# numtel/ntru-circom

Hardware: AMD Instinct MI355X
Metric: NTRU encrypt+decrypt round trips per second at N=821, q=4096 (higher is better)
Workload: dtype i8

## Files before the change

ntru-circom_amd/csrc/matrix_common.h:

```cpp
#ifndef NTRU_MATRIX_COMMON_H
#define NTRU_MATRIX_COMMON_H

#include "kernels_common.h"

typedef int v4i __attribute__((ext_vector_type(4)));
typedef int v16i __attribute__((ext_vector_type(16)));
typedef unsigned int v2u __attribute__((__vector_size__(2 * sizeof(unsigned int))));
constexpr int ST_AUX = 0;

struct MGeom {
  int N;
  int NT;
  int pitchA;
  int tpitch;
  int ld;
};

enum { M_ENC = 0, M_DEC1 = 1, M_DEC2 = 2, M_DEC1T = 3, M_DEC2P = 4 };

#ifdef NTRU_STAMPS
#define STAMP_SLOTS 24
#define STAMP_BLOCKS 6
static __device__ unsigned long long g_stamps[1024][8][STAMP_BLOCKS][STAMP_SLOTS];
#define STAMP(slot)                                                                                          \
// ... 3 lines not shown
  } while (0)
#define NTRU_STAMPS_READER(name) extern "C" int name(void *dst) { return (int)hipMemcpyFromSymbol(dst, HIP_SYMBOL(g_stamps), sizeof(g_stamps)); }
#else
#define STAMP(slot) do { } while (0)
#define NTRU_STAMPS_READER(name)
#endif


template <class D>
static __device__ __forceinline__ void build_toeplitz_array(u32 *T, const MGeom &g, D digit, int tid, int nthr) {
  const int Y0 = 32 * g.NT - 1;
  for (int x = tid; x < 4 * g.tpitch; x += nthr) {
    const int c = x / g.tpitch, w = x - c * g.tpitch;
    u32 v = 0;
#pragma unroll
    for (int j = 0; j < 4; j++) {
      int idx = (Y0 - (4 * w + c + j)) % g.N;
      idx += idx < 0 ? g.N : 0;
      v |= ((u32)digit(idx) & 0xFFu) << (8 * j);
    }
    T[x] = v;
  }
}

static __device__ __forceinline__ const u32 *frag_lane_base(const u32 *T, const MGeom &g, int lane) {
  const int y0 = 32 * g.NT - 1 - (lane & 31) + 16 * (lane >> 5);
  return T + (y0 & 3) * g.tpitch + (y0 >> 2);
}

static __device__ __forceinline__ v4i and4(v4i a, const u32 (&m)[4]) {
  return (v4i){(int)((u32)a[0] & m[0]), (int)((u32)a[1] & m[1]), (int)((u32)a[2] & m[2]), (int)((u32)a[3] & m[3])};
}

struct NoPause { __device__ __forceinline__ void operator()() const {} };
struct NoDiag { __device__ __forceinline__ void operator()(int) const {} };
template <int MODE, int NT_S, class Epi, class Pause = NoPause, class Diag = NoDiag>
static __device__ __forceinline__ void toeplitz_strip(const unsigned char *__restrict__ st0,
                                                      const unsigned char *__restrict__ st1,
                                                      const u32 *__restrict__ tb0, const u32 *__restrict__ tb1,
                                                      const MGeom &g, int kb0, const u32 (&mlow)[4], Epi epi,
                                                      int stamp_iter = 0, int stamp_base = 0, int pause_ib = 0x7fffffff,
                                                      Pause pause = Pause(), Diag diag = Diag(), int ash = 0) {
  constexpr bool TWO = MODE != M_DEC2 && MODE != M_DEC2P;
  v16i accL[NT_S], accH[NT_S];
  v4i W0[NT_S], W1[NT_S];
  auto load_w = [&](int d, v4i &w0, v4i &w1) {
    const u32 *p = tb0 - 8 * d;
    w0 = (v4i){(int)p[0], (int)p[1], (int)p[2], (int)p[3]};
    if (MODE == M_ENC || MODE == M_DEC1T) {
      const u32 *p1 = tb1 - 8 * d;
      w1 = (v4i){(int)p1[0], (int)p1[1], (int)p1[2], (int)p1[3]};
    } else if (MODE == M_DEC1) {
#pragma unroll
      for (int c = 0; c < 4; c++) w1[c] = (int)(((u32)w0[c] << 6) & 0xC0C0C0C0u);
    } else {
      w1 = w0;
    }
  };
  auto load_a = [&](int ib, v4i &a0, v4i &a1) {
    a0 = *(const v4i *)(st0 + 32 * ib);
    if (MODE == M_ENC) {
#pragma unroll
      for (int c = 0; c < 4; c++) a1[c] = (int)((u32)a0[c] << 5);
    } else if (MODE == M_DEC1 || MODE == M_DEC1T) {
      a1 = *(const v4i *)(st1 + 32 * ib);
    } else {
      a1 = a0;
    }
  };
  auto unpack_a = [&](v4i &a0, v4i &a1) {
    if (MODE == M_DEC2P) {
#pragma unroll
      for (int c = 0; c < 4; c++) a0[c] = (int)(((u32)a0[c] >> ash) & 0x03030303u);
      a1 = a0;
    }
  };
  auto mm = [&](v16i &acc, v4i a0, v4i a1, v4i w0, v4i w1) {
    acc = __builtin_amdgcn_mfma_i32_32x32x32_i8(a0, w0, acc, 0, 0, 0);
    if (TWO) acc = __builtin_amdgcn_mfma_i32_32x32x32_i8(a1, w1, acc, 0, 0, 0);
  };
  auto mm_first = [&](v16i &acc, v4i a0, v4i a1, v4i w0, v4i w1) {
    const v16i zero = {0, 0, 0, 0, 0, 0, 0, 0, 0, 0, 0, 0, 0, 0, 0, 0};
    acc = __builtin_amdgcn_mfma_i32_32x32x32_i8(a0, w0, zero, 0, 0, 0);
    if (TWO) acc = __builtin_amdgcn_mfma_i32_32x32x32_i8(a1, w1, acc, 0, 0, 0);
  };
#pragma unroll
  for (int t = 0; t < NT_S; t++) load_w(kb0 + t, W0[t], W1[t]);
  u32 mhigh[4];
#pragma unroll
  for (int c = 0; c < 4; c++) mhigh[c] = ~mlow[c];
  v4i a0, a1;
  load_a(0, a0, a1);
  unpack_a(a0, a1);
  auto block = [&](int ib, auto kind) {
#pragma unroll
    for (int u = 0; u < NT_S; u++) {
      v4i n0, n1;
      load_a(ib + u + 1, n0, n1);
#pragma unroll
      for (int tt = 1; tt <= NT_S; tt++) {
        const int t = tt % NT_S;
        constexpr int K = decltype(kind)::value;
        const int sl = (t - u + NT_S) % NT_S;
        if (K == 0 || (K == 2 && t > u)) mm(accL[t], a0, a1, W0[sl], W1[sl]);
        else if (K == 1 || (K == 2 && t < u)) mm(accH[t], a0, a1, W0[sl], W1[sl]);
        else {
          mm(accL[t], a0, a1, and4(W0[sl], mlow), and4(W1[sl], mlow));
          mm_first(accH[t], a0, a1, and4(W0[sl], mhigh), and4(W1[sl], mhigh));
        }
      }
      load_w(kb0 - (ib + u + 1), W0[(NT_S - 1 - u) % NT_S], W1[(NT_S - 1 - u) % NT_S]);
      if (decltype(kind)::value == 2) diag(u);
      a0 = n0; a1 = n1;
      unpack_a(a0, a1);
    }
  };
  auto single = [&](int ib, v16i (&acc)[NT_S]) {
    v4i n0, n1;
    load_a(ib + 1, n0, n1);
#pragma unroll
    for (int t = 0; t < NT_S; t++) mm(acc[t], a0, a1, W0[t], W1[t]);
#pragma unroll
    for (int t = NT_S - 1; t > 0; t--) { W0[t] = W0[t - 1]; W1[t] = W1[t - 1]; }
    load_w(kb0 - (ib + 1), W0[0], W1[0]);
    a0 = n0; a1 = n1;
    unpack_a(a0, a1);
  };
  int ib = 0;
  bool paused = false;
  if (kb0 > 0 && g.NT > 0) {
    if (!std::is_same<Pause, NoPause>::value && pause_ib <= 0) { pause(); paused = true; load_a(0, a0, a1); unpack_a(a0, a1); }
    v4i n0, n1;
    load_a(1, n0, n1);
#pragma unroll
    for (int t = 0; t < NT_S; t++) mm_first(accL[t], a0, a1, W0[t], W1[t]);
#pragma unroll
    for (int t = NT_S - 1; t > 0; t--) { W0[t] = W0[t - 1]; W1[t] = W1[t - 1]; }
    load_w(kb0 - 1, W0[0], W1[0]);
    a0 = n0; a1 = n1;
    unpack_a(a0, a1);
    ib = 1;
  } else {
#pragma unroll
    for (int t = 0; t < NT_S; t++)
#pragma unroll
      for (int i = 0; i < 16; i++) accL[t][i] = 0;
  }
  auto maybe_pause = [&](int first, int last) {
    if (!std::is_same<Pause, NoPause>::value && !paused && last >= pause_ib) {
      __builtin_amdgcn_s_setprio(0);
      pause();
      __builtin_amdgcn_s_setprio(3);
      paused = true;
      load_a(first, a0, a1);
      unpack_a(a0, a1);
    }
  };
  __builtin_amdgcn_s_setprio(3);
  for (; ib + NT_S <= kb0; ib += NT_S) { maybe_pause(ib, ib + NT_S - 1); block(ib, std::integral_constant<int, 0>{}); }
  for (; ib < kb0; ib++) { maybe_pause(ib, ib); single(ib, accL); }
  maybe_pause(kb0, kb0 + NT_S - 1);
  block(kb0, std::integral_constant<int, 2>{});
  for (ib = kb0 + NT_S; ib + NT_S <= g.NT; ib += NT_S) { maybe_pause(ib, ib + NT_S - 1); block(ib, std::integral_constant<int, 1>{}); }
  for (; ib < g.NT; ib++) { maybe_pause(ib, ib); single(ib, accH); }
  __builtin_amdgcn_s_setprio(0);
  if (!std::is_same<Pause, NoPause>::value && !paused) pause();
  STAMP(stamp_base);
  epi(accL, accH);
  STAMP(stamp_base + 1);
}

template <int MAXT = 4, class Body>
static __device__ __forceinline__ void for_each_strip(int NT, int wave, Body body, bool all = false) {
  const int rounds = (((NT + MAXT - 1) / MAXT) + WAVES_PER_BLOCK - 1) / WAVES_PER_BLOCK;
  const int n_str = rounds * WAVES_PER_BLOCK, base = NT / n_str, rem = NT % n_str;
  if (!all && 2 * blockIdx.x >= gridDim.x) wave ^= 2;
  for (int rho = 0; rho < rounds; rho++) {
    const int j = rho * WAVES_PER_BLOCK + wave;
    const int nt = base + (j < rem ? 1 : 0);
    if (nt > 0 || all) body(j * base + (j < rem ? j : rem), nt);
  }
}

static __device__ __forceinline__ void diag_low_mask(int lane, u32 (&mlow)[4]) {
  const int r = lane & 31, hh = lane >> 5;
#pragma unroll
  for (int c = 0; c < 4; c++) {
    u32 mk = 0;
#pragma unroll
    for (int jj = 0; jj < 4; jj++) mk |= (r >= 16 * hh + 4 * c + jj) ? (0xFFu << (8 * jj)) : 0u;
    mlow[c] = mk;
  }
}

static __device__ __forceinline__ __amdgpu_buffer_rsrc_t rows_rsrc(const void *p, long bytes) {
  const unsigned long long a = (unsigned long long)p;
  const u32 lo = __builtin_amdgcn_readfirstlane((u32)a), hi = __builtin_amdgcn_readfirstlane((u32)(a >> 32));
  const int n = __builtin_amdgcn_readfirstlane((int)(bytes < 0x7FFFF000L ? bytes : 0x7FFFF000L));
  return __builtin_amdgcn_make_buffer_rsrc((void *)(((unsigned long long)hi << 32) | lo), 0, n, 0x00020000);
}
// ... 58 lines not shown
```

ntru-circom_amd/csrc/matrix_decrypt.hip:

```cpp
#include "matrix_common.h"

template <int GROUPS, bool PACK = false>
static __device__ __forceinline__ void decrypt_m_body(MGeom g, u32 q, u32 p, const int8_t *__restrict__ f,
                                                      const uint8_t *__restrict__ fp,
                                                      const u16 *__restrict__ e, long B,
                                                      uint8_t *__restrict__ value, u16 *__restrict__ quot1,
                                                      u16 *__restrict__ rem1, uint8_t *__restrict__ quot2,
                                                      unsigned long long *__restrict__ packed = nullptr, int pack_os = 0) {
  extern __shared__ __attribute__((aligned(16))) unsigned char lds[];
  const int group = GROUPS == 2 ? __builtin_amdgcn_readfirstlane((int)(threadIdx.x >> 8)) : 0;
  static_assert(!PACK || GROUPS == 1, "fused packOutput is built on the plain four-wave kernel");
  const int M3V = __builtin_amdgcn_readfirstlane(((int)((p - 1) * (p - 1)) * g.N + 4) & ~3);
  const int m3_bytes = GROUPS == 2 ? (M3V + (int)((p - 1) * (p - 1)) * g.N + 1 + 15) & ~15 : 0;
  const int gbytes = 64 * g.pitchA + 256 * g.NT;
  unsigned char *stHi = lds + (GROUPS == 2 ? __builtin_amdgcn_readfirstlane(m3_bytes + group * gbytes) : 0);
  unsigned char *stLo = stHi + 32 * g.pitchA;
  unsigned char *blp = stLo + 32 * g.pitchA;
  u32 *TF = (u32 *)(lds + m3_bytes + GROUPS * gbytes), *TP = TF + 4 * g.tpitch, *TF64 = TP + 4 * g.tpitch;
  unsigned char *lift_lut = (unsigned char *)(TP + 4 * g.tpitch * GROUPS);
  const int pcols = 126 * pack_os + 16, pimg_bytes = (8 * pcols + 15) & ~15;
  unsigned char *pimg = stHi + ((((int)((p - 1) * (p - 1)) * g.N + 4) & ~3) + (int)((p - 1) * (p - 1)) * g.N + 1 + 15 & ~15);
  auto pack_flush = [&](long rbx) {
    const long b0x = rbx << 5;
    const int rows_left = (int)(B - b0x < 32 ? B - b0x : 32);
// ... 82 lines not shown
      u32 cmask[8];
#pragma unroll
      for (int c = 0; c < 8; c++) {
        const int left2 = N - (16 * c16 + 2 * c);
        cmask[c] = qm2 & (left2 >= 2 ? 0xFFFFFFFFu : (left2 == 1 ? 0x0000FFFFu : 0u));
      }
#pragma unroll
      for (int j = 0; j < RPW; j++) {
        const int row = wave + WAVES_PER_BLOCK * j;
        v4i v[2];
        shift_raw<2>(raw[j], sh[j], v);
        u32 x[8];
#pragma unroll
        for (int c = 0; c < 4; c++) { x[c] = (u32)v[0][c]; x[4 + c] = (u32)v[1][c]; }
        u32 lo[4], hi[4];
#pragma unroll
        for (int c = 0; c < 4; c++) {
          const u32 xa = x[2 * c] & cmask[2 * c], xb = x[2 * c + 1] & cmask[2 * c + 1];
          lo[c] = __builtin_amdgcn_perm(xb & 0x007F007Fu, xa & 0x007F007Fu, 0x06040200u);
          hi[c] = __builtin_amdgcn_perm((xb >> 6) & 0x00FE00FEu, (xa >> 6) & 0x00FE00FEu, 0x06040200u);
        }
        if (c16 < nch) {
          *(uint4 *)(stLo + row * g.pitchA + 16 * c16) = make_uint4(lo[0], lo[1], lo[2], lo[3]);
          *(uint4 *)(stHi + row * g.pitchA + 16 * c16) = make_uint4(hi[0], hi[1], hi[2], hi[3]);
        }
      }
    }
    STAMP(2);
    __syncthreads();
    STAMP(3);
    const int lane_off = (lane >> 5) * 4 * LD + (lane & 31);
    sidx = 0;
    constexpr int P1 = GROUPS == 2 ? M_DEC1T : M_DEC1;
    for_each_strip<4>(g.NT, GROUPS == 2 ? wave ^ (2 * group) ^ (2 * blockIdx.x >= gridDim.x ? 2 : 0) : wave, [&](int kb0, int nt) {
      auto epi = [&](auto &lo, auto &hi) {
        constexpr int NTS = sizeof(lo) / sizeof(lo[0]);
        phase();
        long bb = b0;
        asm volatile("" : "+s"(bb));
        const long lf = (B - bb) * LD;
        const __amdgpu_buffer_rsrc_t rs_r1 = rows_rsrc(want_r1 ? rem1 + bb * LD : nullptr, want_r1 ? 2 * lf : 0);
        const __amdgpu_buffer_rsrc_t rs_q1 = rows_rsrc(want_q1 ? quot1 + bb * LD : nullptr, want_q1 ? 2 * lf : 0);
        int voff[NTS];
#pragma unroll
        for (int t = 0; t < NTS; t++) voff[t] = 32 * (kb0 + t) + (lane & 31) < N ? 2 * lane_off : (int)0x80000000;
        auto out = [&](auto wr, auto wq) {
#pragma unroll
          for (int j = 0; j < 4; j++) {
            u32 xs[NTS][4], lv[NTS][4];
#pragma unroll
            for (int ii = 0; ii < 4; ii++) {
              const int i = 4 * j + ii, ro = ii + 8 * j;
#pragma unroll
              for (int t = 0; t < NTS; t++) {
                const u32 x = (u32)(lo[t][i] + hi[t][i]) & (q - 1);
                xs[t][ii] = x;
                const int so = 2 * (ro * LD + 32 * (kb0 + t));
                {
                  if (decltype(wr)::value) __builtin_amdgcn_raw_buffer_store_b16((u16)x, rs_r1, voff[t], so, ST_AUX);
                  if (decltype(wq)::value) __builtin_amdgcn_raw_buffer_store_b16((u16)((u32)(0 - hi[t][i]) & (q - 1)), rs_q1, voff[t], so, ST_AUX);
                }
              }
            }
#pragma unroll
            for (int t = 0; t < NTS; t++)
#pragma unroll
              for (int ii = 0; ii < 4; ii++) lv[t][ii] = lift_lut[xs[t][ii]];
#pragma unroll
            for (int t = 0; t < NTS; t++) {
              const int col = 32 * (kb0 + t) + (lane & 31);
              const u32 pk = lv[t][0] | (lv[t][1] << 2) | (lv[t][2] << 4) | (lv[t][3] << 6);
              blp[((lane >> 5) + 2 * j) * 32 * g.NT + col] = (unsigned char)(col < N ? pk : 0u);
            }
          }
        };
        if (want_r1 && want_q1) out(std::true_type{}, std::true_type{});
        else if (want_r1) out(std::true_type{}, std::false_type{});
        else if (want_q1) out(std::false_type{}, std::true_type{});
        else out(std::false_type{}, std::false_type{});
      };
      switch (nt) {
        case 0: phase(); break;
        case 1: toeplitz_strip<P1, 1>(st0, st1, tbf, tbf64, g, kb0, mlow, epi, stamp_iter, 4 + 2 * sidx); break;
        case 2: toeplitz_strip<P1, 2>(st0, st1, tbf, tbf64, g, kb0, mlow, epi, stamp_iter, 4 + 2 * sidx); break;
        case 3: toeplitz_strip<P1, 3>(st0, st1, tbf, tbf64, g, kb0, mlow, epi, stamp_iter, 4 + 2 * sidx); break;
        default: toeplitz_strip<P1, 4>(st0, st1, tbf, tbf64, g, kb0, mlow, epi, stamp_iter, 4 + 2 * sidx); break;
      }
      sidx++;
      if (sidx < rounds) phase();
    }, GROUPS == 2);
    __syncthreads();
    STAMP(8);
    if (PACK) pack_wipe();
    if (GROUPS == 1) build_m3(tid0, BLOCK_THREADS, N);
    if (GROUPS == 1) {
      constexpr int RPW = 32 / WAVES_PER_BLOCK;
      u32 pv[RPW][4];
#pragma unroll
      for (int j = 0; j < RPW; j++) {
        const int row = wave + WAVES_PER_BLOCK * j, rgb = 2 * (row >> 3) + ((row >> 2) & 1);
        const u32 *src = (const u32 *)(blp + rgb * 32 * g.NT);
#pragma unroll
        for (int it = 0; it < 4; it++) pv[j][it] = src[(lane + 64 * it) < 8 * g.NT ? lane + 64 * it : 0];
      }
#pragma unroll
      for (int j = 0; j < RPW; j++) {
        const int row = wave + WAVES_PER_BLOCK * j, sh = 2 * (row & 3);
#pragma unroll
        for (int it = 0; it < 4; it++)
          if (lane + 64 * it < 8 * g.NT) *(u32 *)(stLo + row * g.pitchA + 4 * (lane + 64 * it)) = (pv[j][it] >> sh) & 0x03030303u;
      }
    }
    STAMP(9);
    if (GROUPS == 1) __syncthreads();
    STAMP(10);
    constexpr int P2 = GROUPS == 2 ? M_DEC2P : M_DEC2;
    const unsigned char *a2 = GROUPS == 2 ? blp + ((lane & 31) >> 2) * 32 * g.NT + 16 * (lane >> 5) : st0;
    const int ash = 2 * (lane & 3);
    sidx = 0;
// ... 124 lines not shown
```

ntru-circom_amd/csrc/matrix_encrypt.hip:

```cpp
#include "matrix_common.h"

template <int MAXT, bool DMA>
static __device__ __forceinline__ void encrypt_m_body(MGeom g, u32 q, const u16 *__restrict__ h,
                                                      const uint8_t *__restrict__ r,
                                                      const uint8_t *__restrict__ m, long B,
                                                      u16 *__restrict__ e, u16 *__restrict__ quotE) {
  extern __shared__ __attribute__((aligned(16))) unsigned char lds[];
  auto wg_barrier = [&]() {
    if (DMA) asm volatile("s_waitcnt lgkmcnt(0)\n\ts_barrier" ::: "memory");
    else __syncthreads();
  };
  u32 *T0 = (u32 *)lds, *T1 = T0 + 4 * g.tpitch;
  unsigned char *stA = (unsigned char *)(T1 + 4 * g.tpitch);
  unsigned char *mimg = stA + 32 * g.pitchA;
  const int tid0 = threadIdx.x & (BLOCK_THREADS - 1), lane0 = tid0 & 63, wave = __builtin_amdgcn_readfirstlane(tid0 >> 6);
  const int hthr = (int)(q >> 1) - 65;
  auto hs_of = [&](int i) { int hv = (int)(h[i] & (q - 1)); return hv > hthr ? hv - (int)q : hv; };
  if (q <= 4096) {
    build_toeplitz_array(T0, g, [&](int i) { return (int)(h[i] & (q - 1)) & 127; }, (int)threadIdx.x, BLOCK_THREADS);
    build_toeplitz_array(T1, g, [&](int i) { return ((int)(h[i] & (q - 1)) >> 7) * 4; }, (int)threadIdx.x, BLOCK_THREADS);
  } else {
    build_toeplitz_array(T0, g, [&](int i) { const int hs = hs_of(i); return ((hs + 64) & 127) - 64; }, (int)threadIdx.x, BLOCK_THREADS);
    build_toeplitz_array(T1, g, [&](int i) { const int hs = hs_of(i); const int d0 = ((hs + 64) & 127) - 64; return ((hs - d0) >> 7) * 4; }, (int)threadIdx.x, BLOCK_THREADS);
  }
  const bool want_q = quotE != nullptr;
  const long nrb = (B + 31) >> 5;
  int sidx = 0, stamp_iter = -1;
  const long stride = (long)gridDim.x, iters = (nrb + stride - 1) / stride;
  const int rounds = (((g.NT + MAXT - 1) / MAXT) + WAVES_PER_BLOCK - 1) / WAVES_PER_BLOCK;
  auto dma_r = [&](long rbx, int lane) {
    const long b0x = rbx << 5 < B ? rbx << 5 : B;
    const unsigned long long a = (unsigned long long)(r + b0x * g.ld);
    const int a0 = (int)(a & 3);
    const __amdgpu_buffer_rsrc_t rs = rows_rsrc((const void *)(a & ~3ULL), ((B - b0x) * g.ld + a0 + 3) & ~3L);
#pragma unroll
    for (int j = 0; j < 32 / WAVES_PER_BLOCK; j++) {
      const int row = wave + WAVES_PER_BLOCK * j, ro = a0 + row * g.ld;
      if (lane < (((ro & 3) + g.N + 15) >> 4))
        __builtin_amdgcn_raw_ptr_buffer_load_lds(rs, (__attribute__((address_space(3))) void *)(stA + row * g.pitchA), 16,
                                                 (ro & ~3) + 16 * lane, 0, 0, 0);
    }
  };
  auto dma_m = [&](long rbx, int tid) {
    const long b0x = rbx << 5 < B ? rbx << 5 : B;
    const unsigned long long a = (unsigned long long)(m + b0x * g.ld);
    const int a0 = (int)(a & 3);
    const __amdgpu_buffer_rsrc_t rs = rows_rsrc((const void *)(a & ~3ULL), ((B - b0x) * g.ld + a0 + 3) & ~3L);
    const int npc = (a0 + 32 * g.ld + 15) >> 4;
#pragma unroll
    for (int j = 0; j < 8; j++)
      if (tid + j * BLOCK_THREADS < npc)
        __builtin_amdgcn_raw_ptr_buffer_load_lds(rs, (__attribute__((address_space(3))) void *)(mimg + 16 * (wave * 64 + j * BLOCK_THREADS)), 16,
                                                 16 * (tid + j * BLOCK_THREADS), 0, 0, 0);
  };
  if (DMA) {
    dma_r((long)blockIdx.x < nrb ? (long)blockIdx.x : nrb, lane0);
    __builtin_amdgcn_s_waitcnt(0);
  }
  for (long it = 0; it < iters; it++) {
    long rb = (long)blockIdx.x + it * stride;
    rb = rb < nrb ? rb : nrb;
    long rb_next = (long)blockIdx.x + (it + 1) * stride;
    rb_next = rb_next < nrb ? rb_next : nrb;
    stamp_iter++;
    STAMP(0);
    int lane = lane0, N = g.N, LD = g.ld, tid = tid0;
    asm volatile("" : "+v"(lane), "+s"(N), "+s"(LD), "+v"(tid));
    const u32 *tb0 = frag_lane_base(T0, g, lane), *tb1 = frag_lane_base(T1, g, lane);
    const unsigned char *st0 = stA + (lane & 31) * g.pitchA + 16 * (lane >> 5);
    u32 mlow[4];
    diag_low_mask(lane, mlow);
    const long b0 = rb << 5 < B ? rb << 5 : B, left = (B - b0) * LD;
    const AlignedSrc src_r = aligned_src(r + b0 * LD, left), src_m = aligned_src(m + b0 * LD, left);
    constexpr int RPW = 32 / WAVES_PER_BLOCK;
    const int shm = __builtin_amdgcn_readfirstlane(src_m.a0);
    RawChunks<1> in_r[RPW], in_m[8];
    if (!DMA) {
#pragma unroll
      for (int j = 0; j < RPW; j++) {
        const int pos0 = src_r.a0 + (wave + WAVES_PER_BLOCK * j) * LD;
        in_r[j] = load_raw<1>(src_r, pos0 + 16 * lane, 0);
      }
#pragma unroll
      for (int j = 0; j < 8; j++) {
        const int i = tid * 16 + j * BLOCK_THREADS * 16;
        in_m[j] = load_raw<1>(src_m, src_m.a0 + i, 0);
      }
    }
    wg_barrier();
    STAMP(1);
    const int a0m = DMA ? __builtin_amdgcn_readfirstlane((int)((unsigned long long)(m + b0 * LD) & 3)) : 0;
    if (DMA) {
      dma_m(rb, tid);
      const int a0r = (int)((unsigned long long)(r + b0 * LD) & 3);
      const v4i mk = col_mask16(16 * lane, N);
      int s4[RPW];
#pragma unroll
      for (int j = 0; j < RPW; j++) {
        const int row = wave + WAVES_PER_BLOCK * j;
        const unsigned char *slot = stA + row * g.pitchA + 16 * (lane < 2 * g.NT ? lane : 0);
        in_r[j].c[0] = *(const v4i *)slot;
        in_r[j].tail = *(const u32 *)(slot + 16);
        s4[j] = __builtin_amdgcn_readfirstlane((a0r + row * LD) & 3);
      }
// ... 4 lines not shown
        shift_raw<1>(in_r[j], s4[j], v);
        if (lane < 2 * g.NT) *(v4i *)(stA + row * g.pitchA + 16 * lane) = v[0] & mk;
      }
    } else {
      const v4i mk = col_mask16(16 * lane, N);
#pragma unroll
      for (int j = 0; j < RPW; j++) {
        const int row = wave + WAVES_PER_BLOCK * j;
        v4i v[1];
        shift_raw<1>(in_r[j], src_r.a0 + row * LD, v);
        if (lane < 2 * g.NT) *(v4i *)(stA + row * g.pitchA + 16 * lane) = v[0] & mk;
      }
      STAMP(16);
#pragma unroll
      for (int j = 0; j < 8; j++) {
        const int i = tid * 16 + j * BLOCK_THREADS * 16;
        v4i v[1];
        shift_raw<1>(in_m[j], shm, v);
        if (i < 32 * LD) *(v4i *)(mimg + i) = v[0];
      }
    }
    STAMP(2);
    wg_barrier();
    STAMP(3);
    sidx = 0;
    auto epi_sync = [&]() {
      if (!DMA) return;
      if (sidx == 0) __builtin_amdgcn_s_waitcnt((7 << 4) | (15 << 8));
      if (sidx == 0 || sidx == rounds - 1) wg_barrier();
      if (sidx == rounds - 1 && it + 1 < iters) dma_r(rb_next, lane);
    };
    const bool dma_now = DMA && it + 1 < iters;
    for_each_strip<MAXT>(g.NT, DMA ? wave ^ (2 * (int)blockIdx.x >= (int)gridDim.x ? 2 : 0) : wave, [&](int kb0, int nt) {
      const int lane_off = (lane >> 5) * 4 * LD + (lane & 31);
      auto epi = [&](auto &lo, auto &hi) {
        constexpr int NTS = sizeof(lo) / sizeof(lo[0]);
        epi_sync();
        long bb = b0;
        asm volatile("" : "+s"(bb));
        const long lf = (B - bb) * LD;
        const __amdgpu_buffer_rsrc_t rs_e = rows_rsrc(e + bb * LD, 2 * lf);
        const __amdgpu_buffer_rsrc_t rs_q = rows_rsrc(want_q ? quotE + bb * LD : e + bb * LD, 2 * lf);
        const unsigned char *m_l = mimg + a0m + 32 * kb0 + lane_off;
        int voff[NTS];
#pragma unroll
        for (int t = 0; t < NTS; t++) voff[t] = 32 * (kb0 + t) + (lane & 31) < N ? 2 * lane_off : (int)0x80000000;
        const int pv0 = 32 * kb0 + lane;
        auto out = [&](auto wq) {
#pragma unroll
          for (int j = 0; j < 4; j++) {
            u32 mv[NTS][4];
#pragma unroll
            for (int t = 0; t < NTS; t++)
#pragma unroll
              for (int ii = 0; ii < 4; ii++) mv[t][ii] = m_l[(8 * j + ii) * LD + 32 * t];
            u32 ev[NTS][4], qv[NTS][4];
#pragma unroll
            for (int t = 0; t < NTS; t++)
#pragma unroll
              for (int ii = 0; ii < 4; ii++) {
                ev[t][ii] = (u32)(lo[t][4 * j + ii] + hi[t][4 * j + ii] + (int)mv[t][ii]) & (q - 1);
                qv[t][ii] = (u32)(0 - hi[t][4 * j + ii]) & (q - 1);
              }
#pragma unroll
            for (int t = 0; t + 1 < NTS; t += 2) {
              const int pvoff = pv0 + 32 * t < N ? 2 * lane : (int)0x80000000;
#pragma unroll
              for (int ii = 0; ii < 4; ii++) {
                const auto se = __builtin_amdgcn_permlane32_swap(ev[t][ii], ev[t + 1][ii], false, false);
                const int so = 2 * ((8 * j + ii) * LD + 32 * (kb0 + t));
                {
                  __builtin_amdgcn_raw_buffer_store_b16((u16)se[0], rs_e, pvoff, so, ST_AUX);
                  __builtin_amdgcn_raw_buffer_store_b16((u16)se[1], rs_e, pvoff, so + 8 * LD, ST_AUX);
                  if (decltype(wq)::value) {
                    const auto sq = __builtin_amdgcn_permlane32_swap(qv[t][ii], qv[t + 1][ii], false, false);
                    __builtin_amdgcn_raw_buffer_store_b16((u16)sq[0], rs_q, pvoff, so, ST_AUX);
                    __builtin_amdgcn_raw_buffer_store_b16((u16)sq[1], rs_q, pvoff, so + 8 * LD, ST_AUX);
                  }
                }
              }
            }
            if (NTS & 1) {
              constexpr int t = NTS - 1;
              const int so = 2 * (8 * j * LD + 32 * (kb0 + t));
              {
#pragma unroll
                for (int ii = 0; ii < 4; ii++) {
                  __builtin_amdgcn_raw_buffer_store_b16((u16)ev[t][ii], rs_e, voff[t], so + 2 * ii * LD, ST_AUX);
                  if (decltype(wq)::value) __builtin_amdgcn_raw_buffer_store_b16((u16)qv[t][ii], rs_q, voff[t], so + 2 * ii * LD, ST_AUX);
                }
              }
            }
          }
          constexpr int S = 16 * NTS * (decltype(wq)::value ? 2 : 1), K = S < 63 ? S : 63;
          if (DMA && dma_now && sidx == rounds - 1) __builtin_amdgcn_s_waitcnt((K & 15) | (7 << 4) | (15 << 8) | ((K >> 4) << 14));
        };
        if (want_q) out(std::true_type{}); else out(std::false_type{});
      };
      switch (nt) {
        case 0:
          epi_sync();
          if (DMA && sidx == rounds - 1) __builtin_amdgcn_s_waitcnt((7 << 4) | (15 << 8));
          break;
        case 1: toeplitz_strip<M_ENC, 1>(st0, st0, tb0, tb1, g, kb0, mlow, epi, stamp_iter, 4 + 2 * sidx); break;
        case 2: toeplitz_strip<M_ENC, 2>(st0, st0, tb0, tb1, g, kb0, mlow, epi, stamp_iter, 4 + 2 * sidx); break;
        case 3: toeplitz_strip<M_ENC, 3>(st0, st0, tb0, tb1, g, kb0, mlow, epi, stamp_iter, 4 + 2 * sidx); break;
        case 4: toeplitz_strip<M_ENC, 4>(st0, st0, tb0, tb1, g, kb0, mlow, epi, stamp_iter, 4 + 2 * sidx); break;
        default: break;
      }
      sidx++;
    }, DMA);
  }
}

__global__ __launch_bounds__(BLOCK_THREADS, 2) void k_encrypt_m(MGeom g, u32 q, const u16 *__restrict__ h,
                                                             const uint8_t *__restrict__ r,
                                                             const uint8_t *__restrict__ m, long B,
                                                             u16 *__restrict__ e, u16 *__restrict__ quotE) {
  encrypt_m_body<4, false>(g, q, h, r, m, B, e, quotE);
}

__global__ __launch_bounds__(BLOCK_THREADS, 2) void k_encrypt_md(MGeom g, u32 q, const u16 *__restrict__ h,
                                                              const uint8_t *__restrict__ r,
                                                              const uint8_t *__restrict__ m, long B,
                                                              u16 *__restrict__ e, u16 *__restrict__ quotE) {
  encrypt_m_body<4, true>(g, q, h, r, m, B, e, quotE);
}

NTRU_STAMPS_READER(ntru_debug_read_stamps_enc)

int ntru_launch_encrypt_matrix(ntru_engine *eng, int N, int q, int ld, const uint16_t *d_h, const uint8_t *d_r, const uint8_t *d_m,
                               int64_t B, uint16_t *d_e, uint16_t *d_quotE) {
  MGeom mg;
  if (!make_mgeom(eng, N, q, ld, &mg)) return NTRU_NOT_TAKEN;
  const size_t lds = (size_t)32 * mg.tpitch + (size_t)32 * mg.pitchA + (((size_t)32 * ld + 15) & ~(size_t)15) + 16;
  const long nrb = (long)((B + 31) / 32);
  if (lds > 160 * 1024) return NTRU_NOT_TAKEN;
  const bool rows_dword_aligned = (ld & 3) == 0 && ((uintptr_t)d_r & 3) == 0, img_dword_aligned = (ld & 3) == 0 && ((uintptr_t)d_m & 3) == 0;
  const bool dma_fits = (N + 3 <= 1024 || (rows_dword_aligned && N <= 1024)) && (32 * ld + 3 <= 32768 || (img_dword_aligned && 32 * ld <= 32768));
  const bool md = eng->path != 4 && dma_fits;
  snprintf(eng->last_kernel, sizeof eng->last_kernel, md ? "k_encrypt_md" : "k_encrypt_m");
  return launch_resident(eng, md ? k_encrypt_md : k_encrypt_m, nrb, BLOCK_THREADS, lds, mg, (u32)q, d_h, d_r, d_m, (long)B, d_e, d_quotE);
}
```

Before: 275.8 million.

## Add 16x16x64 MFMA tile form to Toeplitz strip and use it in grouped decrypt

Adds a T16 variant of the Toeplitz strip that issues four 16x16x64 int8 MFMAs per step instead of two 32x32x32 ones. It uses lane-dependent stage and key-fragment bases, a per-lane triangular diagonal mask and a permlane16 swap before the epilogue to restore the row layout. The epilogues are generalized for the new row mapping. The two-group decrypt path now uses this form, while the encrypt kernels keep the 32x32 form. A standalone microbenchmark compares the two MFMA shapes for throughput and power.

```diff
diff --git a/bench_micro/mfma_shape_energy.hip b/bench_micro/mfma_shape_energy.hip
--- /dev/null
+++ b/bench_micro/mfma_shape_energy.hip
@@ -0,0 +1,124 @@
+#include <hip/hip_runtime.h>
+#include <cstdio>
+#include <cstdlib>
+#include <cstring>
+#include <vector>
+#define CK(x) do { hipError_t e_ = (x); if (e_ != hipSuccess) { printf("HIP error %s at %d\n", hipGetErrorString(e_), __LINE__); exit(1);} } while (0)
+typedef int v4i __attribute__((ext_vector_type(4)));
+typedef int v16i __attribute__((ext_vector_type(16)));
+constexpr int PITCH = 32 * 26 + 16, NSTEP = 24;
+constexpr int A_BYTES = 64 * PITCH, T_DW = 1024, LDS_BYTES = A_BYTES + 2 * 4 * T_DW;
+
+template <int SHAPE>
+__global__ __launch_bounds__(512) void k_spin(unsigned long long ticks, const int *__restrict__ in, unsigned long long *out) {
+  __shared__ __attribute__((aligned(16))) unsigned char lds[LDS_BYTES];
+  for (int i = threadIdx.x; i < LDS_BYTES / 4; i += 512) ((int *)lds)[i] = in[i];
+  __syncthreads();
+  const int lane = threadIdx.x & 63;
+  const unsigned *T0 = (const unsigned *)(lds + A_BYTES), *T1 = T0 + T_DW;
+  v4i W[4][2];
+  unsigned long long it = 0;
+  int s = 0;
+  const unsigned long long r0 = __builtin_amdgcn_s_memrealtime(), t0 = __builtin_amdgcn_s_memtime();
+  unsigned long long r1 = r0;
+  if (SHAPE == 32) {
+    const unsigned char *st0 = lds + (lane & 31) * PITCH + 16 * (lane >> 5), *st1 = st0 + 32 * PITCH;
+    const int y0 = 47 - (lane & 31) + 16 * (lane >> 5);
+    const unsigned *tb0 = T0 + (y0 & 3) * 264 + 208 + (y0 >> 2), *tb1 = T1 + (y0 & 3) * 264 + 208 + (y0 >> 2);
+    v16i acc[4];
+    for (int t = 0; t < 4; t++) for (int g = 0; g < 16; g++) acc[t][g] = 0;
+    auto load_w = [&](int d, v4i (&w)[2]) {
+      const unsigned *p = tb0 - 8 * d, *p1 = tb1 - 8 * d;
+      w[0] = (v4i){(int)p[0], (int)p[1], (int)p[2], (int)p[3]};
+      w[1] = (v4i){(int)p1[0], (int)p1[1], (int)p1[2], (int)p1[3]};
+    };
+    while (r1 - r0 < ticks) {
+      for (int t = 0; t < 4; t++) load_w(t, W[t]);
+      for (int ib = 0; ib < NSTEP; ib += 4) {
+#pragma unroll
+        for (int u = 0; u < 4; u++) {
+          const v4i a0 = *(const v4i *)(st0 + 32 * (ib + u)), a1 = *(const v4i *)(st1 + 32 * (ib + u));
+#pragma unroll
+          for (int tt = 1; tt <= 4; tt++) {
+            const int t = tt % 4, sl = (t - u + 4) % 4;
+            acc[t] = __builtin_amdgcn_mfma_i32_32x32x32_i8(a0, W[sl][0], acc[t], 0, 0, 0);
+            acc[t] = __builtin_amdgcn_mfma_i32_32x32x32_i8(a1, W[sl][1], acc[t], 0, 0, 0);
+          }
+          load_w(ib + u + 1, W[(3 - u) % 4]);
+        }
+      }
+      it += NSTEP;
+      r1 = __builtin_amdgcn_s_memrealtime();
+    }
+    for (int t = 0; t < 4; t++) for (int g = 0; g < 16; g++) s ^= acc[t][g];
+  } else {
+    const int kq = lane >> 4;
+    const unsigned char *st = lds + (kq >> 1) * 32 * PITCH + (lane & 15) * PITCH + 16 * (kq & 1);
+    const int y0 = 47 - (lane & 15) + 16 * (kq & 1);
+    const unsigned *tb = ((kq >> 1) ? T1 : T0) + (y0 & 3) * 264 + 208 + (y0 >> 2);
+    v4i acc[4][2][2];
+    for (int t = 0; t < 4; t++) for (int g = 0; g < 4; g++) acc[t][0][0][g] = acc[t][0][1][g] = acc[t][1][0][g] = acc[t][1][1][g] = 0;
+    auto load_w = [&](int d, v4i (&w)[2]) {
+      const unsigned *p = tb - 8 * d;
+      w[0] = (v4i){(int)p[0], (int)p[1], (int)p[2], (int)p[3]};
+      w[1] = (v4i){(int)p[-4], (int)p[-3], (int)p[-2], (int)p[-1]};
+    };
+    while (r1 - r0 < ticks) {
+      for (int t = 0; t < 4; t++) load_w(t, W[t]);
+      for (int ib = 0; ib < NSTEP; ib += 4) {
+#pragma unroll
+        for (int u = 0; u < 4; u++) {
+          const v4i a0 = *(const v4i *)(st + 32 * (ib + u)), a1 = *(const v4i *)(st + 32 * (ib + u) + 16 * PITCH);
+#pragma unroll
+          for (int tt = 1; tt <= 4; tt++) {
+            const int t = tt % 4, sl = (t - u + 4) % 4;
+            acc[t][0][0] = __builtin_amdgcn_mfma_i32_16x16x64_i8(a0, W[sl][0], acc[t][0][0], 0, 0, 0);
+            acc[t][0][1] = __builtin_amdgcn_mfma_i32_16x16x64_i8(a0, W[sl][1], acc[t][0][1], 0, 0, 0);
+            acc[t][1][0] = __builtin_amdgcn_mfma_i32_16x16x64_i8(a1, W[sl][0], acc[t][1][0], 0, 0, 0);
+            acc[t][1][1] = __builtin_amdgcn_mfma_i32_16x16x64_i8(a1, W[sl][1], acc[t][1][1], 0, 0, 0);
+          }
+          load_w(ib + u + 1, W[(3 - u) % 4]);
+        }
+      }
+      it += NSTEP;
+      r1 = __builtin_amdgcn_s_memrealtime();
+    }
+    for (int t = 0; t < 4; t++) for (int g = 0; g < 4; g++) s ^= acc[t][0][0][g] ^ acc[t][0][1][g] ^ acc[t][1][0][g] ^ acc[t][1][1][g];
+  }
+  const unsigned long long t1 = __builtin_amdgcn_s_memtime();
+  if (lane == 0) {
+    const int w = blockIdx.x * 8 + (threadIdx.x >> 6);
+    out[3 * w] = it + (s == 0x7fffffff); out[3 * w + 1] = t1 - t0; out[3 * w + 2] = r1 - r0;
+  }
+}
+
+int main(int argc, char **argv) {
+  const char *arm = argc > 1 ? argv[1] : "32";
+  const int shape = atoi(arm);
+  const bool zero = strchr(arm, 'z') != nullptr;
+  const double seconds = argc > 2 ? atof(argv[2]) : 3.0;
+  if (shape != 32 && shape != 16) { printf("arm: 32, 16, 32z or 16z\n"); return 2; }
+  CK(hipSetDevice(0));
+  hipDeviceProp_t prop; CK(hipGetDeviceProperties(&prop, 0));
+  char pci[64]; CK(hipDeviceGetPCIBusId(pci, sizeof pci, 0));
+  printf("pci_bus_id %s\n", pci);
+  std::vector<int> h(LDS_BYTES / 4);
+  unsigned x = 7; for (auto &v : h) { x = x * 1664525u + 1013904223u; v = zero ? 0 : (int)(x ^ (x >> 13)); }
+  int *d_in; unsigned long long *d_out;
+  const int blocks = prop.multiProcessorCount;
+  CK(hipMalloc(&d_in, LDS_BYTES)); CK(hipMemcpy(d_in, h.data(), LDS_BYTES, hipMemcpyHostToDevice));
+  CK(hipMalloc(&d_out, (size_t)blocks * 8 * 3 * 8));
+  const unsigned long long ticks = (unsigned long long)(seconds * 1e8);
+  if (shape == 32) hipLaunchKernelGGL(k_spin<32>, dim3(blocks), dim3(512), 0, 0, ticks, d_in, d_out);
+  else hipLaunchKernelGGL(k_spin<16>, dim3(blocks), dim3(512), 0, 0, ticks, d_in, d_out);
+  CK(hipGetLastError());
+  CK(hipDeviceSynchronize());
+  std::vector<unsigned long long> o((size_t)blocks * 8 * 3);
+  CK(hipMemcpy(o.data(), d_out, o.size() * 8, hipMemcpyDeviceToHost));
+  double steps = 0, clk = 0, ref = 0;
+  for (int w = 0; w < blocks * 8; w++) { steps += (double)o[3 * w]; clk += (double)o[3 * w + 1]; ref += (double)o[3 * w + 2]; }
+  const double secs = ref / (blocks * 8) / 1e8, sets = steps * 8;
+  printf("arm %s: %.4e sets of 32768 MACs in %.2f s = %.3f G sets/s; %.1f wave clocks per step; shader clock %.3f GHz\n", arm, sets, secs,
+         sets / secs / 1e9, clk / steps, clk / ref * 0.1);
+  return 0;
+}
diff --git a/ntru-circom_amd/csrc/matrix_common.h b/ntru-circom_amd/csrc/matrix_common.h
--- a/ntru-circom_amd/csrc/matrix_common.h
+++ b/ntru-circom_amd/csrc/matrix_common.h
@@ -59,9 +59,30 @@
   return (v4i){(int)((u32)a[0] & m[0]), (int)((u32)a[1] & m[1]), (int)((u32)a[2] & m[2]), (int)((u32)a[3] & m[3])};
 }
 
+struct Tile16 { v4i q[4]; };
+static __device__ __forceinline__ int acc_at(const v16i &t, int i) { return t[i]; }
+static __device__ __forceinline__ int acc_at(const Tile16 &t, int i) { return t.q[i >> 2][i & 3]; }
+template <bool T16> constexpr int tile_half_rows() { return T16 ? 8 : 4; }
+template <bool T16> constexpr int tile_row4(int jq) { return T16 ? 16 * (jq >> 1) + 4 * (jq & 1) : 8 * jq; }
+
+static __device__ __forceinline__ const unsigned char *tile16_stage(const unsigned char *stage0, const unsigned char *stage1, const MGeom &g, int lane) {
+  return ((lane & 32) ? stage1 : stage0) + (lane & 15) * g.pitchA + (lane & 16);
+}
+static __device__ __forceinline__ const u32 *tile16_frag_base(const u32 *T0, const u32 *T1, const MGeom &g, int lane) {
+  return frag_lane_base((lane & 32) ? T1 : T0, g, (lane & 15) + 2 * (lane & 16));
+}
+static __device__ __forceinline__ void tile16_tri(int lane, u32 (&tri)[4]) {
+  const int m = lane & 15;
+#pragma unroll
+  for (int c = 0; c < 4; c++) {
+    const int n = m - 4 * c + 1;
+    tri[c] = n <= 0 ? 0u : ~0u >> (n >= 4 ? 0 : 32 - 8 * n);
+  }
+}
+
 struct NoPause { __device__ __forceinline__ void operator()() const {} };
 struct NoDiag { __device__ __forceinline__ void operator()(int) const {} };
-template <int MODE, int NT_S, class Epi, class Pause = NoPause, class Diag = NoDiag>
+template <int MODE, int NT_S, bool T16 = false, class Epi, class Pause = NoPause, class Diag = NoDiag>
 static __device__ __forceinline__ void toeplitz_strip(const unsigned char *__restrict__ st0,
                                                       const unsigned char *__restrict__ st1,
                                                       const u32 *__restrict__ tb0, const u32 *__restrict__ tb1,
@@ -69,12 +90,16 @@
                                                       int stamp_iter = 0, int stamp_base = 0, int pause_ib = 0x7fffffff,
                                                       Pause pause = Pause(), Diag diag = Diag(), int ash = 0) {
   constexpr bool TWO = MODE != M_DEC2 && MODE != M_DEC2P;
-  v16i accL[NT_S], accH[NT_S];
+  static_assert(!T16 || MODE == M_ENC || MODE == M_DEC1T, "the 16-row tile form carries two planes read from two key arrays");
+  typedef typename std::conditional<T16, Tile16, v16i>::type Acc;
+  Acc accL[NT_S], accH[NT_S];
   v4i W0[NT_S], W1[NT_S];
   auto load_w = [&](int d, v4i &w0, v4i &w1) {
     const u32 *p = tb0 - 8 * d;
     w0 = (v4i){(int)p[0], (int)p[1], (int)p[2], (int)p[3]};
-    if (MODE == M_ENC || MODE == M_DEC1T) {
+    if (T16) {
+      w1 = (v4i){(int)p[-4], (int)p[-3], (int)p[-2], (int)p[-1]};
+    } else if (MODE == M_ENC || MODE == M_DEC1T) {
       const u32 *p1 = tb1 - 8 * d;
       w1 = (v4i){(int)p1[0], (int)p1[1], (int)p1[2], (int)p1[3]};
     } else if (MODE == M_DEC1) {
@@ -86,7 +111,13 @@
   };
   auto load_a = [&](int ib, v4i &a0, v4i &a1) {
     a0 = *(const v4i *)(st0 + 32 * ib);
-    if (MODE == M_ENC) {
+    if (T16) {
+      a1 = *(const v4i *)(st0 + 32 * ib + 16 * g.pitchA);
+      if (MODE == M_ENC) {
+#pragma unroll
+        for (int c = 0; c < 4; c++) { a0[c] = (int)((u32)a0[c] << ash); a1[c] = (int)((u32)a1[c] << ash); }
+      }
+    } else if (MODE == M_ENC) {
 #pragma unroll
       for (int c = 0; c < 4; c++) a1[c] = (int)((u32)a0[c] << 5);
     } else if (MODE == M_DEC1 || MODE == M_DEC1T) {
@@ -102,20 +133,51 @@
       a1 = a0;
     }
   };
-  auto mm = [&](v16i &acc, v4i a0, v4i a1, v4i w0, v4i w1) {
-    acc = __builtin_amdgcn_mfma_i32_32x32x32_i8(a0, w0, acc, 0, 0, 0);
-    if (TWO) acc = __builtin_amdgcn_mfma_i32_32x32x32_i8(a1, w1, acc, 0, 0, 0);
-  };
-  auto mm_first = [&](v16i &acc, v4i a0, v4i a1, v4i w0, v4i w1) {
-    const v16i zero = {0, 0, 0, 0, 0, 0, 0, 0, 0, 0, 0, 0, 0, 0, 0, 0};
-    acc = __builtin_amdgcn_mfma_i32_32x32x32_i8(a0, w0, zero, 0, 0, 0);
-    if (TWO) acc = __builtin_amdgcn_mfma_i32_32x32x32_i8(a1, w1, acc, 0, 0, 0);
+  auto mm = [&](Acc &acc, v4i a0, v4i a1, v4i w0, v4i w1) {
+    if constexpr (T16) {
+      acc.q[0] = __builtin_amdgcn_mfma_i32_16x16x64_i8(a0, w0, acc.q[0], 0, 0, 0);
+      acc.q[1] = __builtin_amdgcn_mfma_i32_16x16x64_i8(a0, w1, acc.q[1], 0, 0, 0);
+      acc.q[2] = __builtin_amdgcn_mfma_i32_16x16x64_i8(a1, w0, acc.q[2], 0, 0, 0);
+      acc.q[3] = __builtin_amdgcn_mfma_i32_16x16x64_i8(a1, w1, acc.q[3], 0, 0, 0);
+    } else {
+      acc = __builtin_amdgcn_mfma_i32_32x32x32_i8(a0, w0, acc, 0, 0, 0);
+      if (TWO) acc = __builtin_amdgcn_mfma_i32_32x32x32_i8(a1, w1, acc, 0, 0, 0);
+    }
+  };
+  auto mm_first = [&](Acc &acc, v4i a0, v4i a1, v4i w0, v4i w1) {
+    if constexpr (T16) {
+      const v4i zero = {0, 0, 0, 0};
+      acc.q[0] = __builtin_amdgcn_mfma_i32_16x16x64_i8(a0, w0, zero, 0, 0, 0);
+      acc.q[1] = __builtin_amdgcn_mfma_i32_16x16x64_i8(a0, w1, zero, 0, 0, 0);
+      acc.q[2] = __builtin_amdgcn_mfma_i32_16x16x64_i8(a1, w0, zero, 0, 0, 0);
+      acc.q[3] = __builtin_amdgcn_mfma_i32_16x16x64_i8(a1, w1, zero, 0, 0, 0);
+    } else {
+      const v16i zero = {0, 0, 0, 0, 0, 0, 0, 0, 0, 0, 0, 0, 0, 0, 0, 0};
+      acc = __builtin_amdgcn_mfma_i32_32x32x32_i8(a0, w0, zero, 0, 0, 0);
+      if (TWO) acc = __builtin_amdgcn_mfma_i32_32x32x32_i8(a1, w1, acc, 0, 0, 0);
+    }
+  };
+  u32 mhigh[4];
+#pragma unroll
+  for (int c = 0; c < 4; c++) mhigh[c] = ~mlow[c];
+  auto mm_diag = [&](Acc &aL, Acc &aH, v4i a0, v4i a1, v4i w0, v4i w1) {
+    if constexpr (T16) {
+      u32 z = 0;
+      asm volatile("" : "+v"(z));
+      const u32 m0 = (__builtin_amdgcn_mbcnt_hi(~0u, __builtin_amdgcn_mbcnt_lo(~0u, z)) & 16u) ? 0u : ~0u;
+      u32 l0[4], l1[4];
+#pragma unroll
+      for (int c = 0; c < 4; c++) { l0[c] = mlow[c] & m0; l1[c] = mlow[c] | m0; }
+      const v4i wl0 = and4(w0, l0), wl1 = and4(w1, l1);
+      mm(aL, a0, a1, wl0, wl1);
+      mm_first(aH, a0, a1, w0 ^ wl0, w1 ^ wl1);
+    } else {
+      mm(aL, a0, a1, and4(w0, mlow), and4(w1, mlow));
+      mm_first(aH, a0, a1, and4(w0, mhigh), and4(w1, mhigh));
+    }
   };
 #pragma unroll
   for (int t = 0; t < NT_S; t++) load_w(kb0 + t, W0[t], W1[t]);
-  u32 mhigh[4];
-#pragma unroll
-  for (int c = 0; c < 4; c++) mhigh[c] = ~mlow[c];
   v4i a0, a1;
   load_a(0, a0, a1);
   unpack_a(a0, a1);
@@ -131,10 +193,7 @@
         const int sl = (t - u + NT_S) % NT_S;
         if (K == 0 || (K == 2 && t > u)) mm(accL[t], a0, a1, W0[sl], W1[sl]);
         else if (K == 1 || (K == 2 && t < u)) mm(accH[t], a0, a1, W0[sl], W1[sl]);
-        else {
-          mm(accL[t], a0, a1, and4(W0[sl], mlow), and4(W1[sl], mlow));
-          mm_first(accH[t], a0, a1, and4(W0[sl], mhigh), and4(W1[sl], mhigh));
-        }
+        else mm_diag(accL[t], accH[t], a0, a1, W0[sl], W1[sl]);
       }
       load_w(kb0 - (ib + u + 1), W0[(NT_S - 1 - u) % NT_S], W1[(NT_S - 1 - u) % NT_S]);
       if (decltype(kind)::value == 2) diag(u);
@@ -142,7 +201,7 @@
       unpack_a(a0, a1);
     }
   };
-  auto single = [&](int ib, v16i (&acc)[NT_S]) {
+  auto single = [&](int ib, Acc (&acc)[NT_S]) {
     v4i n0, n1;
     load_a(ib + 1, n0, n1);
 #pragma unroll
@@ -169,9 +228,12 @@
     ib = 1;
   } else {
 #pragma unroll
-    for (int t = 0; t < NT_S; t++)
-#pragma unroll
-      for (int i = 0; i < 16; i++) accL[t][i] = 0;
+    for (int t = 0; t < NT_S; t++) {
+      if constexpr (T16) accL[t].q[0] = accL[t].q[1] = accL[t].q[2] = accL[t].q[3] = (v4i){0, 0, 0, 0};
+      else
+#pragma unroll
+        for (int i = 0; i < 16; i++) accL[t][i] = 0;
+    }
   }
   auto maybe_pause = [&](int first, int last) {
     if (!std::is_same<Pause, NoPause>::value && !paused && last >= pause_ib) {
@@ -193,6 +255,19 @@
   __builtin_amdgcn_s_setprio(0);
   if (!std::is_same<Pause, NoPause>::value && !paused) pause();
   STAMP(stamp_base);
+  if constexpr (T16) {
+#pragma unroll
+    for (int t = 0; t < NT_S; t++)
+#pragma unroll
+      for (int rh = 0; rh < 2; rh++)
+#pragma unroll
+        for (int j = 0; j < 4; j++) {
+          const auto sl = __builtin_amdgcn_permlane16_swap((u32)accL[t].q[2 * rh][j], (u32)accL[t].q[2 * rh + 1][j], false, false);
+          accL[t].q[2 * rh][j] = (int)sl[0]; accL[t].q[2 * rh + 1][j] = (int)sl[1];
+          const auto sh = __builtin_amdgcn_permlane16_swap((u32)accH[t].q[2 * rh][j], (u32)accH[t].q[2 * rh + 1][j], false, false);
+          accH[t].q[2 * rh][j] = (int)sh[0]; accH[t].q[2 * rh + 1][j] = (int)sh[1];
+        }
+  }
   epi(accL, accH);
   STAMP(stamp_base + 1);
 }
diff --git a/ntru-circom_amd/csrc/matrix_decrypt.hip b/ntru-circom_amd/csrc/matrix_decrypt.hip
--- a/ntru-circom_amd/csrc/matrix_decrypt.hip
+++ b/ntru-circom_amd/csrc/matrix_decrypt.hip
@@ -138,6 +138,15 @@
     const int lane_off = (lane >> 5) * 4 * LD + (lane & 31);
     sidx = 0;
     constexpr int P1 = GROUPS == 2 ? M_DEC1T : M_DEC1;
+    constexpr bool T16 = GROUPS == 2;
+    constexpr int HR = tile_half_rows<T16>();
+    const unsigned char *sa1 = T16 ? tile16_stage(stLo, stHi, g, lane) : st0;
+    const u32 *tb1 = T16 ? tile16_frag_base(TF, TF64, g, lane) : tbf;
+    u32 mlow1[4];
+    if (T16) tile16_tri(lane, mlow1);
+    else
+#pragma unroll
+      for (int c = 0; c < 4; c++) mlow1[c] = mlow[c];
     for_each_strip<4>(g.NT, GROUPS == 2 ? wave ^ (2 * group) ^ (2 * blockIdx.x >= gridDim.x ? 2 : 0) : wave, [&](int kb0, int nt) {
       auto epi = [&](auto &lo, auto &hi) {
         constexpr int NTS = sizeof(lo) / sizeof(lo[0]);
@@ -149,22 +158,22 @@
         const __amdgpu_buffer_rsrc_t rs_q1 = rows_rsrc(want_q1 ? quot1 + bb * LD : nullptr, want_q1 ? 2 * lf : 0);
         int voff[NTS];
 #pragma unroll
-        for (int t = 0; t < NTS; t++) voff[t] = 32 * (kb0 + t) + (lane & 31) < N ? 2 * lane_off : (int)0x80000000;
+        for (int t = 0; t < NTS; t++) voff[t] = 32 * (kb0 + t) + (lane & 31) < N ? 2 * ((lane >> 5) * HR * LD + (lane & 31)) : (int)0x80000000;
         auto out = [&](auto wr, auto wq) {
 #pragma unroll
           for (int j = 0; j < 4; j++) {
             u32 xs[NTS][4], lv[NTS][4];
 #pragma unroll
             for (int ii = 0; ii < 4; ii++) {
-              const int i = 4 * j + ii, ro = ii + 8 * j;
+              const int i = 4 * j + ii, ro = ii + tile_row4<T16>(j);
 #pragma unroll
               for (int t = 0; t < NTS; t++) {
-                const u32 x = (u32)(lo[t][i] + hi[t][i]) & (q - 1);
+                const u32 x = (u32)(acc_at(lo[t], i) + acc_at(hi[t], i)) & (q - 1);
                 xs[t][ii] = x;
                 const int so = 2 * (ro * LD + 32 * (kb0 + t));
                 {
                   if (decltype(wr)::value) __builtin_amdgcn_raw_buffer_store_b16((u16)x, rs_r1, voff[t], so, ST_AUX);
-                  if (decltype(wq)::value) __builtin_amdgcn_raw_buffer_store_b16((u16)((u32)(0 - hi[t][i]) & (q - 1)), rs_q1, voff[t], so, ST_AUX);
+                  if (decltype(wq)::value) __builtin_amdgcn_raw_buffer_store_b16((u16)((u32)(0 - acc_at(hi[t], i)) & (q - 1)), rs_q1, voff[t], so, ST_AUX);
                 }
               }
             }
@@ -176,7 +185,8 @@
             for (int t = 0; t < NTS; t++) {
               const int col = 32 * (kb0 + t) + (lane & 31);
               const u32 pk = lv[t][0] | (lv[t][1] << 2) | (lv[t][2] << 4) | (lv[t][3] << 6);
-              blp[((lane >> 5) + 2 * j) * 32 * g.NT + col] = (unsigned char)(col < N ? pk : 0u);
+              const int rg = T16 ? 4 * (j >> 1) + (j & 1) + 2 * (lane >> 5) : (lane >> 5) + 2 * j;
+              blp[rg * 32 * g.NT + col] = (unsigned char)(col < N ? pk : 0u);
             }
           }
         };
@@ -187,10 +197,10 @@
       };
       switch (nt) {
         case 0: phase(); break;
-        case 1: toeplitz_strip<P1, 1>(st0, st1, tbf, tbf64, g, kb0, mlow, epi, stamp_iter, 4 + 2 * sidx); break;
-        case 2: toeplitz_strip<P1, 2>(st0, st1, tbf, tbf64, g, kb0, mlow, epi, stamp_iter, 4 + 2 * sidx); break;
-        case 3: toeplitz_strip<P1, 3>(st0, st1, tbf, tbf64, g, kb0, mlow, epi, stamp_iter, 4 + 2 * sidx); break;
-        default: toeplitz_strip<P1, 4>(st0, st1, tbf, tbf64, g, kb0, mlow, epi, stamp_iter, 4 + 2 * sidx); break;
+        case 1: toeplitz_strip<P1, 1, T16>(sa1, st1, tb1, tbf64, g, kb0, mlow1, epi, stamp_iter, 4 + 2 * sidx); break;
+        case 2: toeplitz_strip<P1, 2, T16>(sa1, st1, tb1, tbf64, g, kb0, mlow1, epi, stamp_iter, 4 + 2 * sidx); break;
+        case 3: toeplitz_strip<P1, 3, T16>(sa1, st1, tb1, tbf64, g, kb0, mlow1, epi, stamp_iter, 4 + 2 * sidx); break;
+        default: toeplitz_strip<P1, 4, T16>(sa1, st1, tb1, tbf64, g, kb0, mlow1, epi, stamp_iter, 4 + 2 * sidx); break;
       }
       sidx++;
       if (sidx < rounds) phase();
diff --git a/ntru-circom_amd/csrc/matrix_encrypt.hip b/ntru-circom_amd/csrc/matrix_encrypt.hip
--- a/ntru-circom_amd/csrc/matrix_encrypt.hip
+++ b/ntru-circom_amd/csrc/matrix_encrypt.hip
@@ -1,6 +1,6 @@
 #include "matrix_common.h"
 
-template <int MAXT, bool DMA>
+template <int MAXT, bool DMA, bool T16>
 static __device__ __forceinline__ void encrypt_m_body(MGeom g, u32 q, const u16 *__restrict__ h,
                                                       const uint8_t *__restrict__ r,
                                                       const uint8_t *__restrict__ m, long B,
@@ -66,10 +66,11 @@
     STAMP(0);
     int lane = lane0, N = g.N, LD = g.ld, tid = tid0;
     asm volatile("" : "+v"(lane), "+s"(N), "+s"(LD), "+v"(tid));
-    const u32 *tb0 = frag_lane_base(T0, g, lane), *tb1 = frag_lane_base(T1, g, lane);
-    const unsigned char *st0 = stA + (lane & 31) * g.pitchA + 16 * (lane >> 5);
+    const u32 *tb0 = T16 ? tile16_frag_base(T0, T1, g, lane) : frag_lane_base(T0, g, lane), *tb1 = T16 ? tb0 : frag_lane_base(T1, g, lane);
+    const unsigned char *st0 = T16 ? tile16_stage(stA, stA, g, lane) : stA + (lane & 31) * g.pitchA + 16 * (lane >> 5);
+    const int ash = T16 ? (lane & 32 ? 5 : 0) : 0;
     u32 mlow[4];
-    diag_low_mask(lane, mlow);
+    if (T16) tile16_tri(lane, mlow); else diag_low_mask(lane, mlow);
     const long b0 = rb << 5 < B ? rb << 5 : B, left = (B - b0) * LD;
     const AlignedSrc src_r = aligned_src(r + b0 * LD, left), src_m = aligned_src(m + b0 * LD, left);
     constexpr int RPW = 32 / WAVES_PER_BLOCK;
@@ -140,7 +141,8 @@
     };
     const bool dma_now = DMA && it + 1 < iters;
     for_each_strip<MAXT>(g.NT, DMA ? wave ^ (2 * (int)blockIdx.x >= (int)gridDim.x ? 2 : 0) : wave, [&](int kb0, int nt) {
-      const int lane_off = (lane >> 5) * 4 * LD + (lane & 31);
+      constexpr int HR = tile_half_rows<T16>();
+      const int lane_off = (lane >> 5) * HR * LD + (lane & 31);
       auto epi = [&](auto &lo, auto &hi) {
         constexpr int NTS = sizeof(lo) / sizeof(lo[0]);
         epi_sync();
@@ -161,14 +163,14 @@
 #pragma unroll
             for (int t = 0; t < NTS; t++)
 #pragma unroll
-              for (int ii = 0; ii < 4; ii++) mv[t][ii] = m_l[(8 * j + ii) * LD + 32 * t];
+              for (int ii = 0; ii < 4; ii++) mv[t][ii] = m_l[(tile_row4<T16>(j) + ii) * LD + 32 * t];
             u32 ev[NTS][4], qv[NTS][4];
 #pragma unroll
             for (int t = 0; t < NTS; t++)
 #pragma unroll
               for (int ii = 0; ii < 4; ii++) {
-                ev[t][ii] = (u32)(lo[t][4 * j + ii] + hi[t][4 * j + ii] + (int)mv[t][ii]) & (q - 1);
-                qv[t][ii] = (u32)(0 - hi[t][4 * j + ii]) & (q - 1);
+                ev[t][ii] = (u32)(acc_at(lo[t], 4 * j + ii) + acc_at(hi[t], 4 * j + ii) + (int)mv[t][ii]) & (q - 1);
+                qv[t][ii] = (u32)(0 - acc_at(hi[t], 4 * j + ii)) & (q - 1);
               }
 #pragma unroll
             for (int t = 0; t + 1 < NTS; t += 2) {
@@ -176,21 +178,21 @@
 #pragma unroll
               for (int ii = 0; ii < 4; ii++) {
                 const auto se = __builtin_amdgcn_permlane32_swap(ev[t][ii], ev[t + 1][ii], false, false);
-                const int so = 2 * ((8 * j + ii) * LD + 32 * (kb0 + t));
+                const int so = 2 * ((tile_row4<T16>(j) + ii) * LD + 32 * (kb0 + t));
                 {
                   __builtin_amdgcn_raw_buffer_store_b16((u16)se[0], rs_e, pvoff, so, ST_AUX);
-                  __builtin_amdgcn_raw_buffer_store_b16((u16)se[1], rs_e, pvoff, so + 8 * LD, ST_AUX);
+                  __builtin_amdgcn_raw_buffer_store_b16((u16)se[1], rs_e, pvoff, so + 2 * HR * LD, ST_AUX);
                   if (decltype(wq)::value) {
                     const auto sq = __builtin_amdgcn_permlane32_swap(qv[t][ii], qv[t + 1][ii], false, false);
                     __builtin_amdgcn_raw_buffer_store_b16((u16)sq[0], rs_q, pvoff, so, ST_AUX);
-                    __builtin_amdgcn_raw_buffer_store_b16((u16)sq[1], rs_q, pvoff, so + 8 * LD, ST_AUX);
+                    __builtin_amdgcn_raw_buffer_store_b16((u16)sq[1], rs_q, pvoff, so + 2 * HR * LD, ST_AUX);
                   }
                 }
               }
             }
             if (NTS & 1) {
               constexpr int t = NTS - 1;
-              const int so = 2 * (8 * j * LD + 32 * (kb0 + t));
+              const int so = 2 * (tile_row4<T16>(j) * LD + 32 * (kb0 + t));
               {
 #pragma unroll
                 for (int ii = 0; ii < 4; ii++) {
@@ -210,10 +212,10 @@
           epi_sync();
           if (DMA && sidx == rounds - 1) __builtin_amdgcn_s_waitcnt((7 << 4) | (15 << 8));
           break;
-        case 1: toeplitz_strip<M_ENC, 1>(st0, st0, tb0, tb1, g, kb0, mlow, epi, stamp_iter, 4 + 2 * sidx); break;
-        case 2: toeplitz_strip<M_ENC, 2>(st0, st0, tb0, tb1, g, kb0, mlow, epi, stamp_iter, 4 + 2 * sidx); break;
-        case 3: toeplitz_strip<M_ENC, 3>(st0, st0, tb0, tb1, g, kb0, mlow, epi, stamp_iter, 4 + 2 * sidx); break;
-        case 4: toeplitz_strip<M_ENC, 4>(st0, st0, tb0, tb1, g, kb0, mlow, epi, stamp_iter, 4 + 2 * sidx); break;
+        case 1: toeplitz_strip<M_ENC, 1, T16>(st0, st0, tb0, tb1, g, kb0, mlow, epi, stamp_iter, 4 + 2 * sidx, 0x7fffffff, NoPause(), NoDiag(), ash); break;
+        case 2: toeplitz_strip<M_ENC, 2, T16>(st0, st0, tb0, tb1, g, kb0, mlow, epi, stamp_iter, 4 + 2 * sidx, 0x7fffffff, NoPause(), NoDiag(), ash); break;
+        case 3: toeplitz_strip<M_ENC, 3, T16>(st0, st0, tb0, tb1, g, kb0, mlow, epi, stamp_iter, 4 + 2 * sidx, 0x7fffffff, NoPause(), NoDiag(), ash); break;
+        case 4: toeplitz_strip<M_ENC, 4, T16>(st0, st0, tb0, tb1, g, kb0, mlow, epi, stamp_iter, 4 + 2 * sidx, 0x7fffffff, NoPause(), NoDiag(), ash); break;
         default: break;
       }
       sidx++;
@@ -225,14 +227,14 @@
                                                              const uint8_t *__restrict__ r,
                                                              const uint8_t *__restrict__ m, long B,
                                                              u16 *__restrict__ e, u16 *__restrict__ quotE) {
-  encrypt_m_body<4, false>(g, q, h, r, m, B, e, quotE);
+  encrypt_m_body<4, false, false>(g, q, h, r, m, B, e, quotE);
 }
 
 __global__ __launch_bounds__(BLOCK_THREADS, 2) void k_encrypt_md(MGeom g, u32 q, const u16 *__restrict__ h,
                                                               const uint8_t *__restrict__ r,
                                                               const uint8_t *__restrict__ m, long B,
                                                               u16 *__restrict__ e, u16 *__restrict__ quotE) {
-  encrypt_m_body<4, true>(g, q, h, r, m, B, e, quotE);
+  encrypt_m_body<4, true, false>(g, q, h, r, m, B, e, quotE);
 }
 
 NTRU_STAMPS_READER(ntru_debug_read_stamps_enc)
```

After: 272.8 million. -1.1%, worse.
